# shangzhouye/stereo-visual-slam

Hardware: AMD Instinct MI355X
Metric: stereo keyframes/sec (ORB+match+tri+local-BA), KITTI-00 1241x376 (higher is better)
Workload: dtype u8+f64

## Files before the change

### stereo-visual-slam_amd/csrc/api.hip

```cpp
#include <stdarg.h>
#include <stdlib.h>

#include <algorithm>
#include <cmath>
#include <cfloat>
#include <cmath>
#include <vector>

#include "se3_device.h"
#include "vslam_internal.h"

#include <mutex>

namespace vslam {

static thread_local char g_err[512] = "";
void set_error(const char* fmt, ...) {
    va_list ap;
    va_start(ap, fmt);
    vsnprintf(g_err, sizeof(g_err), fmt, ap);
    va_end(ap);
}

struct Prof {
// ... 48 lines not shown
    c->stage_bytes = want; c->dev_bytes += want;
    return VSLAM_OK;
}
template <typename T>
static T* arena_take(Arena& a, size_t n) {
    a.off = (a.off + 255) & ~(size_t)255;
    T* p = reinterpret_cast<T*>(a.c->d_stage + a.off);
    a.off += n * sizeof(T);
    return p;
}
static size_t al256(size_t x) { return (x + 255) & ~(size_t)255; }

static CamParams cam_of(const Ctx* c) {
    CamParams cam;
    cam.fx = c->p.cam[0]; cam.fy = c->p.cam[1]; cam.cx = c->p.cam[2]; cam.cy = c->p.cam[3]; cam.b = c->p.cam[4];
    cam.dmin = c->p.depth_min; cam.dmax = c->p.depth_max; cam.drel = c->p.depth_reliable; cam.row_tol = c->p.stereo_row_tol;
    return cam;
}

template <typename T>
static int dev_alloc(Ctx* c, T** p, size_t n) {
    VS_HIP(hipMalloc((void**)p, n * sizeof(T)));
    c->dev_bytes += n * sizeof(T);
    return VSLAM_OK;
}

struct TuneKey { const char* name; const char* env; int Tuning::*field; int lo, hi; };
static const TuneKey kTuneKeys[] = {
    {"orb_fuse_min", "VSLAM_ORB_FUSE_MIN", &Tuning::orb_fuse_min, 0, 1 << 30},
    {"sgbm_fuse_min", "VSLAM_SGBM_FUSE_MIN", &Tuning::sgbm_fuse_min, 0, 1 << 30},
    {"sgbm_fwd_min", "VSLAM_SGBM_FWD_MIN", &Tuning::sgbm_fwd_min, 0, 1 << 30},
    {"sgbm_fw_rows", "VSLAM_SGBM_FW_ROWS", &Tuning::sgbm_fw_rows, 32, 64},
    {"pose_only_window", "VSLAM_POSE_ONLY_WINDOW", &Tuning::pose_only_window, 0, 1},
    {"ba_resident", "VSLAM_BA_RESIDENT", &Tuning::ba_resident, 0, 1},
    {"pnp_window", "VSLAM_PNP_WINDOW", &Tuning::pnp_window, 0, 1},
    {"ba_adaptive", "VSLAM_BA_ADAPTIVE", &Tuning::ba_adaptive, 0, 1},
    {"ba_lanes", "VSLAM_BA_LANES", &Tuning::ba_lanes, 256, 512},
    {"track_rule", "VSLAM_TRACK_RULE", &Tuning::track_rule, 0, 1},
};
static int tune_set(Tuning& t, const TuneKey& k, long v) {
    if (v == -1) { t.*(k.field) = -1; return VSLAM_OK; }
    if (v < k.lo || v > k.hi || (k.field == &Tuning::sgbm_fw_rows && v != 32 && v != 64) || (k.field == &Tuning::ba_lanes && v != 256 && v != 512)) {
        set_error("tuning value %s = %ld out of range (%d..%d%s, or -1 = default)", k.name, v, k.lo, k.hi, k.field == &Tuning::sgbm_fw_rows ? ", 32 or 64" : "");
        return VSLAM_ERR_ARG;
    }
    t.*(k.field) = (int)v;
    return VSLAM_OK;
}
static int tune_from_env(Tuning& t) {
    for (const TuneKey& k : kTuneKeys) {
        const char* e = getenv(k.env);
        if (!e || !*e) continue;
        char* end = nullptr;
        const long v = strtol(e, &end, 10);
        if (end == e || *end != 0) { set_error("environment variable %s = \"%s\" is not an integer", k.env, e); return VSLAM_ERR_ARG; }
        int rc = tune_set(t, k, v);
        if (rc) return rc;
    }
    return VSLAM_OK;
}

static int orb_status_check(Ctx* c, int B) {
    std::vector<int32_t> st(B);
    VS_HIP(hipMemcpyAsync(st.data(), c->orb.d_status, sizeof(int32_t) * B, hipMemcpyDeviceToHost, c->stream));
    VS_HIP(hipStreamSynchronize(c->stream));
    for (int b = 0; b < B; ++b)
// ... 1042 lines not shown
```

### stereo-visual-slam_amd/csrc/lm_kernels.hip

```cpp
#include "vslam_internal.h"

#include <stdlib.h>

#include <vector>

#include "se3_device.h"
#include "lm_device.h"

namespace vslam {

constexpr int kLmBlock = 512;
constexpr int kLmItemFixed = 128;
constexpr int kLmMinWaves = 2;
constexpr int kLmWaves = kLmBlock / 64;
constexpr int kMaxKf = VSLAM_MAX_KF;
constexpr int kMaxNp = 6 * kMaxKf;
constexpr int kMaxPairs = kMaxKf * (kMaxKf + 1) / 2;
constexpr int kHitsPerEdge = (kMaxKf + 1) / 2 + 1;
constexpr int kDinvLds = 1950;
constexpr int kLin = 2;
constexpr int kPoseParts = 3;
constexpr int kCntStride = 80;
constexpr int kItemSlots = (kMaxPairs + kLmWaves - 1) / kLmWaves;
constexpr int kDbgSlots = 24;
constexpr int kLmSlots = 5;
constexpr int kSchedFinalIters = 10;
constexpr int kRowCap = 512;

size_t lm_hits_per_edge() { return kHitsPerEdge; }

struct alignas(16) LmShared {
    double S[kMaxNp * kMaxNp];
    double Hpp[kMaxKf * 36], HppT[kMaxKf * 36];
    double bp[kMaxNp], bpT[kMaxNp], bs[kMaxNp], xp[kMaxNp];
    double rdiag[kMaxNp];
    double Ld[kMaxKf * 24];
// ... 4 lines not shown
    int ptot[kCntStride];
    int cnt[kLmWaves * kCntStride];
    uint8_t item[kLmWaves * kItemSlots];
    uint8_t pk1[kCntStride], pk2[kCntStride];
    int kfp[kMaxKf + 4];
    int rowp[kMaxKf + 4];
    int flag[8];
    int pairp[kMaxPairs + 2];
    uint8_t rowmax[kRowCap];
};
static_assert(kMaxKf * kPoseParts >= kMaxKf + kLmWaves - 1, "part[] must hold one slot per (keyframe, wave) segment");
static_assert(kLmWaves <= 16, "cnt rows");
static_assert(kMaxNp <= 128, "the backward substitution keeps two unknowns per lane of a wave");
static_assert(kMaxPairs <= kLmWaves * kItemSlots, "item[] too small");

struct LmKernelArgs {
    LmWindowArgs a;
    const int32_t* pnp_n;
    int capacity;
    uint8_t* act;
    int32_t* kf_pos;
    double* chi2k;
    float* uvk;
    int32_t* status;
    long long* dbg_cycles;
    float* slot_uv;
    uint8_t* slot_kf;
    uint8_t* lcnt;
    int dinv_lds;
    int want_chi2;
    const int32_t* order;
    int32_t* passes;
    const int32_t* defer;
};

__device__ inline int slot_width(const uint8_t* rowmax, int first) {
    const int row = first >> 6;
    return __builtin_amdgcn_readfirstlane(row < kRowCap ? (int)rowmax[min(row, kRowCap - 1)] : kLmSlots);
}

__device__ inline double block_sum(double v, double* red) {
    v = wave_sum(v);
    __syncthreads();
    if ((threadIdx.x & 63) == 0) red[threadIdx.x >> 6] = v;
    __syncthreads();
    double s = 0;
    for (int w = 0; w < kLmWaves; ++w) s += red[w];
    return s;
}
__device__ inline double block_max(double v, double* red) {
    v = wave_max(v);
    __syncthreads();
    if ((threadIdx.x & 63) == 0) red[threadIdx.x >> 6] = v;
    __syncthreads();
    double s = red[0];
    for (int w = 1; w < kLmWaves; ++w) s = fmax(s, red[w]);
    return s;
}

template <bool IMPL, bool SCHED = false>
__global__ __launch_bounds__(kLmBlock, kLmMinWaves) void lm_window_kernel(LmKernelArgs ka, int mode, int iters, int update_poses, int update_lms,
                                                            int classify, int reuse_csr) {
    static_assert(!(IMPL && SCHED), "the schedule is a property of the window problems");
    const LmWindowArgs& a = ka.a;
    __shared__ LmShared sm;
    const int w = ka.order ? ka.order[blockIdx.x] : (int)blockIdx.x;
// ... 1158 lines not shown
                currentChi = tempChi;
#pragma unroll
                for (int i = 0; i < 7; ++i) T[i] = Tt[i];
#pragma unroll
                for (int i = 0; i < 12; ++i) Rt[i] = Rtt[i];
            } else {
                lambda *= ni;
                ni *= 2;
            }
            ++qmax;
            again = (rho_gain < 0) && qmax < 10;
        }
        total_trials += qmax;
        if (st && lane == 0 && it < VSLAM_LM_MAX_ITERS) { st->chi2_iter[it] = currentChi; st->lambda_iter[it] = lambda; st->trials_iter[it] = qmax; }
        if (qmax == 10 || rho_gain == 0) { ++it; break; }
    }
    if (st && lane == 0) { st->iterations = it; st->total_trials = total_trials; st->chi2_final = currentChi; st->lambda_final = lambda; }
    if (lane < 7) d_T[7 * (size_t)b + lane] = T[lane];
    int mine = 0;
    for (int i = lane; i < n; i += 64) {
        const size_t gi = (size_t)b * capacity + i;
        double X, Y, Z, ex, ey;
        project_err(Rt, K, (double)px[3 * i], (double)px[3 * i + 1], (double)px[3 * i + 2], uv[2 * gi], uv[2 * gi + 1], X, Y, Z, ex, ey);
        const double c = ex * ex + ey * ey;
        const bool ok = isfinite(c) && c <= thr2;
        if (inlier) inlier[gi] = ok;
        mine += ok;
    }
    for (int o = 32; o > 0; o >>= 1) mine += __shfl_xor(mine, o);
    if (lane == 0 && n_inl) n_inl[b] = mine;
}

constexpr int kPoBlock = 64 * kMaxKf;
struct PoShared {
    double H[2][kMaxKf][36], g[2][kMaxKf][6];
    double part[2][kMaxKf], spart[2][kMaxKf];
    int cnt[kMaxKf][kMaxKf];
    int kbeg[kMaxKf + 1];
    int flag[2];
    int cin[2][kMaxKf], cout[2][kMaxKf];
    double T[2][kMaxKf][7], R[3][kMaxKf][12];
};
__global__ __launch_bounds__(kPoBlock) void pose_only_wave_kernel(LmKernelArgs ka, int iters, int update_poses) {
    const LmWindowArgs& a = ka.a;
    __shared__ PoShared sm;
    const int w = ka.order ? ka.order[blockIdx.x] : (int)blockIdx.x, tid = threadIdx.x, lane = tid & 63;
    const int wave = __builtin_amdgcn_readfirstlane(tid >> 6);
    if (ka.status[w] != VSLAM_OK) return;
    long long* cyc = ka.dbg_cycles ? ka.dbg_cycles + kDbgSlots * (size_t)w : nullptr;
    long long t_ph = cyc ? clock64() : 0;
#define POH(i) do { if (cyc && tid == 0) { const long long t1__ = clock64(); cyc[i] += t1__ - t_ph; t_ph = t1__; } } while (0)
    const int nk = a.n_kf_w ? min(max(a.n_kf_w[w], 1), a.n_kf) : a.n_kf;
    const int lm0 = a.lm_off[w], e0 = a.edge_off[w], ne = a.edge_off[w + 1] - e0;
    const int32_t* kfi = a.kf_idx + e0;
    const int32_t* lmi = a.lm_idx + e0;
    const float2* uv2 = reinterpret_cast<const float2*>(a.uv) + e0;
    const float* xyz = a.xyz + 3 * (size_t)lm0;
    uint8_t* inl = a.lm_inlier + lm0;
    int32_t* list = a.kf_edges + e0;
    float2* uvk = reinterpret_cast<float2*>(ka.uvk) + e0;
    float4* posk = reinterpret_cast<float4*>(a.lin) + e0;
    double* chik = ka.chi2k + e0;
    const double K[4] = {a.K[0], a.K[1], a.K[2], a.K[3]};
    const CamK ck = make_camk(K);
    const double delta = a.huber_delta;
    const unsigned long long lt_mask = (1ull << lane) - 1ull;
    const int per = (((ne + kMaxKf - 1) / kMaxKf) + 63) & ~63;
    const int c0 = min(wave * per, ne), c1 = min(c0 + per, ne);
    {
        int cnt[kMaxKf];
#pragma unroll
        for (int k = 0; k < kMaxKf; ++k) cnt[k] = 0;
        for (int base = c0; base < c1; base += 256) {
            int kq[4], lq[4]; bool vq[4]; uint8_t iq[4];
#pragma unroll
            for (int u = 0; u < 4; ++u) { const int e = base + 64 * u + lane; vq[u] = e < c1; const int es = min(e, ne - 1); kq[u] = kfi[es]; lq[u] = lmi[es]; }
#pragma unroll
            for (int u = 0; u < 4; ++u) iq[u] = inl[lq[u]];
#pragma unroll
            for (int u = 0; u < 4; ++u) {
                const bool act = vq[u] && iq[u] != 0;
#pragma unroll
                for (int kk = 0; kk < kMaxKf; ++kk) cnt[kk] += __popcll(__ballot(act && kq[u] == kk));
            }
        }
        if (lane < kMaxKf) {
            int v = 0;
#pragma unroll
            for (int kk = 0; kk < kMaxKf; ++kk) if (lane == kk) v = cnt[kk];
            sm.cnt[wave][lane] = v;
        }
        if (tid < 2) sm.flag[tid] = 0;
    }
    __syncthreads();
    int off[kMaxKf];
    {
        int run = 0;
#pragma unroll
        for (int k = 0; k < kMaxKf; ++k) {
            int before = 0, tot = 0;
#pragma unroll
            for (int c = 0; c < kMaxKf; ++c) { const int v = sm.cnt[c][k]; tot += v; if (c < wave) before += v; }
            off[k] = run + before;
            if (tid == 0) sm.kbeg[k] = run;
            run += tot;
        }
        if (tid == 0) sm.kbeg[kMaxKf] = run;
    }
    for (int base = c0; base < c1; base += 256) {
        int kq[4], lq[4], eq[4]; bool vq[4]; uint8_t iq[4]; float2 zq[4]; float Xq[4], Yq[4], Zq[4];
#pragma unroll
        for (int u = 0; u < 4; ++u) {
            const int e = base + 64 * u + lane; vq[u] = e < c1; eq[u] = e;
            const int es = min(e, ne - 1);
            kq[u] = kfi[es]; lq[u] = lmi[es]; zq[u] = uv2[es];
        }
#pragma unroll
        for (int u = 0; u < 4; ++u) { iq[u] = inl[lq[u]]; Xq[u] = xyz[3 * lq[u]]; Yq[u] = xyz[3 * lq[u] + 1]; Zq[u] = xyz[3 * lq[u] + 2]; }
#pragma unroll
        for (int u = 0; u < 4; ++u) {
            const bool act = vq[u] && iq[u] != 0;
#pragma unroll
            for (int kk = 0; kk < kMaxKf; ++kk) {
                const unsigned long long m = __ballot(act && kq[u] == kk);
                if (act && kq[u] == kk) {
                    const int pos = off[kk] + __popcll(m & lt_mask);
                    list[pos] = eq[u]; uvk[pos] = zq[u]; posk[pos] = make_float4(Xq[u], Yq[u], Zq[u], 0.f);
                }
                off[kk] += __popcll(m);
            }
        }
    }
    __syncthreads();
    POH(0);
    const int ntot = sm.kbeg[kMaxKf];
    const bool mine = wave < nk;
    const int kb = mine ? sm.kbeg[wave] : 0, ke = mine ? sm.kbeg[wave + 1] : 0;
    {
        double T[7], Rt[12];
#pragma unroll
        for (int i = 0; i < 7; ++i) T[i] = a.T[((size_t)w * a.n_kf + min(wave, nk - 1)) * 7 + i];
        expand_pose(T, Rt);
        if (lane == 0) {
#pragma unroll
            for (int i = 0; i < 7; ++i) sm.T[0][wave][i] = T[i];
#pragma unroll
            for (int i = 0; i < 12; ++i) { sm.R[0][wave][i] = Rt[i]; sm.R[2][wave][i] = Rt[i]; }
        }
        __builtin_amdgcn_wave_barrier();
    }
    const int slot27 = wave_slot<27>(lane);
    auto evaluate = [&](const double* Rlds, bool lin, int buf, bool store_chi) -> double {
        double R[12];
#pragma unroll
        for (int i = 0; i < 12; ++i) R[i] = uniform_f64(Rlds[i]);
        double part = 0, acc[27];
#pragma unroll
        for (int i = 0; i < 27; ++i) acc[i] = 0;
        float4 pp[2], pn[2]; float2 zz[2], zn[2];
#pragma unroll
        for (int u = 0; u < 2; ++u) { const int j = min(kb + 64 * u + lane, max(ke - 1, 0)); pp[u] = posk[j]; zz[u] = uvk[j]; }
        for (int j0 = kb; j0 < ke; j0 += 128) {
#pragma unroll
            for (int u = 0; u < 2; ++u) { const int j = min(j0 + 128 + 64 * u + lane, ke - 1); pn[u] = posk[j]; zn[u] = uvk[j]; }
#pragma unroll
            for (int u = 0; u < 2; ++u) {
                const int j = j0 + 64 * u + lane;
                if (j >= ke) continue;
                double x, y, ri, wgt, ex, ey, c, rho;
                cam_norm(R, (double)pp[u].x, (double)pp[u].y, (double)pp[u].z, x, y, ri);
                eval_obs(ck, x, y, zz[u], delta, ex, ey, c, rho, wgt);
                part += rho;
                if (store_chi) chik[j] = c;
                if (lin) {
                    double A[12], wA[12];
                    jac_norm(x, y, ri, A);
                    const double l0 = wgt * ck.fx2, l1 = wgt * ck.fy2;
#pragma unroll
                    for (int i = 0; i < 6; ++i) { wA[i] = l0 * A[i]; wA[6 + i] = l1 * A[6 + i]; }
                    int idx = 0;
#pragma unroll
                    for (int r = 0; r < 6; ++r)
#pragma unroll
                        for (int cc = r; cc < 6; ++cc) { acc[idx] = a_fma_pair(wA, r, A, cc, acc[idx]); ++idx; }
#pragma unroll
                    for (int r = 0; r < 6; ++r) acc[21 + r] = a_fma2(wA, r, -ex, -ey, acc[21 + r]);
                }
            }
#pragma unroll
            for (int u = 0; u < 2; ++u) { pp[u] = pn[u]; zz[u] = zn[u]; }
        }
        const double total = wave_sum(part);
        if (lin && mine) {
            wave_reduce_scatter<27>(acc, lane);
            if (slot27 >= 0 && slot27 < 21) {
                int r = 0, rem = slot27;
                while (rem >= 6 - r) { rem -= 6 - r; ++r; }
                const int cc = r + rem;
                sm.H[buf][wave][6 * r + cc] = acc[0]; sm.H[buf][wave][6 * cc + r] = acc[0];
            } else if (slot27 >= 21) sm.g[buf][wave][slot27 - 21] = acc[0];
        }
        return total;
    };
    auto sum_kf = [&](const double* v) -> double {
        double t = 0;
        for (int k = 0; k < nk; ++k) t += v[k];
        return t;
    };
    vslam_lm_stats* st = a.stats ? a.stats + w : nullptr;
    double lambda = 0, ni = 2, currentChi = 0;
    int pc = 0;
    int cur = 0, it = 0, total_trials = 0, pb = 0, fb = 0;
    if (iters > 0) {
        const double c = evaluate(sm.R[pc][wave], true, cur, false);
        if (lane == 0 && mine) sm.part[pb][wave] = c;
        __syncthreads();
        currentChi = sum_kf(sm.part[pb]);
        pb ^= 1;
        double md = 0;
        for (int k = 0; k < nk; ++k)
#pragma unroll
            for (int d = 0; d < 6; ++d) md = fmax(md, fabs(sm.H[cur][k][7 * d]));
        lambda = 1e-5 * md;
        if (st && tid == 0) st->chi2_init = currentChi;
    }
    POH(1);
    for (it = 0; it < iters; ++it) {
        double rho_gain = 0;
        int qmax = 0;
        bool again = true;
        while (again) {
            double x[6] = {0, 0, 0, 0, 0, 0};
            if (mine) {
                double Hk[36], gk[6];
#pragma unroll
                for (int i = 0; i < 36; ++i) Hk[i] = sm.H[cur][wave][i];
#pragma unroll
                for (int i = 0; i < 6; ++i) gk[i] = sm.g[cur][wave][i];
                if (!chol6_solve(Hk, lambda, gk, x) && lane == 0) sm.flag[fb] = 1;
            }
            POH(2);
            __syncthreads();
            POH(3);
            const bool ok2 = sm.flag[fb] == 0;
            if (tid == 0) sm.flag[fb ^ 1] = 0;
            fb ^= 1;
            if (!ok2) {
#pragma unroll
                for (int i = 0; i < 6; ++i) x[i] = 0;
            }
            {
                double E[7], Tc[7], Tt[7], Rtt[12];
#pragma unroll
                for (int i = 0; i < 7; ++i) Tc[i] = sm.T[pc][wave][i];
                se3::exp(x, E);
                se3::mul(E, Tc, Tt);
                expand_pose(Tt, Rtt);
                __builtin_amdgcn_wave_barrier();
                if (lane == 0) {
#pragma unroll
                    for (int i = 0; i < 7; ++i) sm.T[pc ^ 1][wave][i] = Tt[i];
#pragma unroll
                    for (int i = 0; i < 12; ++i) { sm.R[pc ^ 1][wave][i] = Rtt[i]; sm.R[2][wave][i] = Rtt[i]; }
                }
                __builtin_amdgcn_wave_barrier();
            }
            POH(4);
            const double c = evaluate(sm.R[pc ^ 1][wave], true, cur ^ 1, false);
            POH(5);
            double sc = 0;
            if (mine) {
#pragma unroll
                for (int i = 0; i < 6; ++i) sc += x[i] * (lambda * x[i] + sm.g[cur][wave][i]);
            }
            if (lane == 0 && mine) { sm.part[pb][wave] = c; sm.spart[pb][wave] = sc; }
            __syncthreads();
            POH(6);
            double tempChi = sum_kf(sm.part[pb]);
            const double scale = sum_kf(sm.spart[pb]) + 1e-3;
            pb ^= 1;
            if (!ok2) tempChi = 1.7976931348623157e308;
            rho_gain = (currentChi - tempChi) / scale;
            if (rho_gain > 0 && isfinite(tempChi)) {
                double alpha = 1. - pow(2 * rho_gain - 1, 3);
                alpha = fmin(alpha, 2. / 3.);
                lambda *= fmax(1. / 3., alpha);
                ni = 2;
                currentChi = tempChi;
                pc ^= 1;
                cur ^= 1;
            } else {
                lambda *= ni;
                ni *= 2;
            }
            ++qmax;
            again = (rho_gain < 0) && qmax < 10;
        }
        total_trials += qmax;
        if (st && tid == 0 && it < VSLAM_LM_MAX_ITERS) { st->chi2_iter[it] = currentChi; st->lambda_iter[it] = lambda; st->trials_iter[it] = qmax; }
        if (qmax == 10 || rho_gain == 0) { ++it; break; }
    }
    if (st && tid == 0) { st->iterations = it; st->total_trials = total_trials; st->chi2_final = currentChi; st->lambda_final = lambda; }
    POH(7);
    evaluate(sm.R[2][wave], false, 0, true);
    double th = delta;
    int cb = 0;
    for (int iteration = 0; iteration < 5; ++iteration) {
        int cin = 0, cout = 0;
        for (int j = kb + lane; j < ke; j += 64) { if (chik[j] > th) ++cout; else ++cin; }
        for (int o = 32; o > 0; o >>= 1) { cin += __shfl_xor(cin, o); cout += __shfl_xor(cout, o); }
        if (lane == 0) { sm.cin[cb][wave] = mine ? cin : 0; sm.cout[cb][wave] = mine ? cout : 0; }
        __syncthreads();
        int tin = 0, tout = 0;
        for (int k = 0; k < nk; ++k) { tin += sm.cin[cb][k]; tout += sm.cout[cb][k]; }
        cb ^= 1;
        const double ratio = (double)tin / (double)(tin + tout);
        if (ratio > 0.5) break;
        th *= 2;
    }
    if (ka.want_chi2) {
        double* chi2 = a.chi2 + e0;
        for (int e = tid; e < ne; e += kPoBlock) if (!inl[lmi[e]]) chi2[e] = 0.0;
        for (int j = kb + lane; j < ke; j += 64) chi2[list[j]] = chik[j];
    }
    __syncthreads();
    for (int j = kb + lane; j < ke; j += 64) {
        const int e = list[j];
        if (e == ne - 1 || lmi[e + 1] != lmi[e]) inl[lmi[e]] = !(chik[j] > th);
    }
    if (tid == 0 && a.chi2_thr) a.chi2_thr[w] = th;
    if (update_poses && mine && lane < 7) a.T[((size_t)w * a.n_kf + wave) * 7 + lane] = sm.T[pc][wave][lane];
    POH(8);
    (void)ntot;
#undef POH
}

static int ensure(void** p, size_t* have, size_t need) {
    if (*have >= need) return VSLAM_OK;
    if (*p) hipFree(*p);
    *p = nullptr; *have = 0;
    if (hipMalloc(p, need) != hipSuccess) { set_error("LM scratch hipMalloc(%zu) failed", need); return VSLAM_ERR_HIP; }
    *have = need;
    return VSLAM_OK;
}

static int carve(LmScratch& g_lm, LmKernelArgs& ka, size_t total_lm, size_t total_edge, int n_windows, bool with_lm, hipStream_t stream) {
    auto al = [](size_t x) { return (x + 255) & ~(size_t)255; };
    size_t need = 0;
    const size_t o_P = need; need += al(total_lm * 3 * 8);
    const size_t o_Pt = need; need += al(total_lm * 3 * 8);
    const size_t o_Hll = need; need += al(total_lm * 6 * 8);
    const size_t o_bl = need; need += al(total_lm * 3 * 8);
    const size_t o_Di = need; need += al(total_lm * 6 * 8);
    const size_t o_lin = need; need += al(total_edge * kLin * 8);
    const size_t o_lmptr = need; need += al((total_lm + n_windows + 1) * 4);
    const size_t o_kfptr = need; need += al((size_t)n_windows * (kMaxKf + 1) * 4);
    const size_t o_kfe = need; need += al(total_edge * 4);
    const size_t o_pp = need; need += al((size_t)n_windows * (kMaxPairs + 1) * 4);
    const size_t o_hits = need; need += with_lm ? al(total_edge * kHitsPerEdge * 8) : 256;
    const size_t o_act = need; need += al(total_lm);
    const size_t o_kpos = need; need += al(total_edge * 4);
    const size_t o_st = need; need += al((size_t)n_windows * 4);
    const size_t o_chi = need; need += al(total_edge * 8);
    const size_t o_chik = need; need += al(total_edge * 8);
    const size_t o_uvk = need; need += al(total_edge * 8);
    const size_t o_suv = need; need += with_lm ? al(total_lm * kLmSlots * 8) : 256;
// ... 83 lines not shown
        L.dyn_bytes = scratch->rs_dyn_bytes; L.schedule = schedule; L.adaptive = adaptive ? 1 : 0; L.iters = iters; L.update_poses = update_poses; L.update_lms = update_lms;
        L.opt_in_done = scratch->rs_opt_in; L.want_chi2 = ka.want_chi2;
        L.dense_to_general = !(scratch->tune && scratch->tune->ba_resident == 1);
        if (schedule && !adaptive) hipLaunchKernelGGL(lm_fill_kernel, dim3((a.n_windows + 255) / 256), dim3(256), 0, stream, ka.passes, a.n_windows, 3);
        rc = launch_ba_resident(L, stream);
        if (rc) return rc;
        scratch->rs_opt_in = true;
        ka.defer = scratch->defer;
        if (L.dbg) {
            hipStreamSynchronize(stream);
            std::vector<long long> h(kDbgSlots * (size_t)a.n_windows);
            hipMemcpy(h.data(), ka.dbg_cycles, sizeof(long long) * h.size(), hipMemcpyDeviceToHost);
            static const char* rs_names[16] = {"setup", "pass init", "boot evaluation", "lambda-init pass", "linearise", "convert+cholesky+solve", "pose update+backsub+trial eval",
                                               "(loop tail)", "classification", "write-back", "lin: row open", "lin: landmark blocks", "lin: diag pair (row-wise)", "lin: off-diag pairs (row-wise)", "lin: singles chunks", "(classification: row loop)"};
            double tot = 0;
            for (int i = 0; i < 16; ++i) { double sum = 0; for (int w = 0; w < a.n_windows; ++w) sum += (double)h[16 * (size_t)w + i]; sum /= a.n_windows; if (i < 10) tot += sum; fprintf(stderr, "  [rs profile] %-32s %10.0f ticks/window\n", rs_names[i], sum); }
            fprintf(stderr, "  [rs profile] total %.0f (clock64 ticks)\n", tot);
            hipMemsetAsync(ka.dbg_cycles, 0, sizeof(long long) * kDbgSlots * a.n_windows, stream);
        }
    }
    if (schedule) {
        if (adaptive) {
            hipLaunchKernelGGL((lm_window_kernel<false, true>), dim3(a.n_windows), dim3(kLmBlock), dyn_lds, stream, ka, 0, 5, 0, 0, 1, 0);
        } else {
            if (!resident) hipLaunchKernelGGL(lm_fill_kernel, dim3((a.n_windows + 255) / 256), dim3(256), 0, stream, ka.passes, a.n_windows, 3);
            hipLaunchKernelGGL(lm_window_kernel<false>, dim3(a.n_windows), dim3(kLmBlock), dyn_lds, stream, ka, 0, 5, 0, 0, 1, 0);
            hipLaunchKernelGGL(lm_window_kernel<false>, dim3(a.n_windows), dim3(kLmBlock), dyn_lds, stream, ka, 0, 5, 0, 0, 1, 1);
            hipLaunchKernelGGL(lm_window_kernel<false>, dim3(a.n_windows), dim3(kLmBlock), dyn_lds, stream, ka, 0, kSchedFinalIters, 1, 0, 1, 1);
        }
        ka.defer = nullptr;
        const bool po_window = scratch->tune && scratch->tune->pose_only_window > 0;
        if (po_window) hipLaunchKernelGGL(lm_window_kernel<false>, dim3(a.n_windows), dim3(kLmBlock), dyn_lds, stream, ka, 1, 10, 1, 0, 1, resident ? 0 : 1);
        else {
            if (ka.dbg_cycles && getenv("VSLAM_PO_PROFILE")) hipMemsetAsync(ka.dbg_cycles, 0, sizeof(long long) * kDbgSlots * a.n_windows, stream);
            hipLaunchKernelGGL(pose_only_wave_kernel, dim3(a.n_windows), dim3(kPoBlock), 0, stream, ka, 10, 1);
        }
    } else {
        hipLaunchKernelGGL(lm_window_kernel<false>, dim3(a.n_windows), dim3(kLmBlock), dyn_lds, stream, ka, mode, iters, update_poses, update_lms, 1, 0);
    }
    VS_HIP(hipGetLastError());
    if (ka.dbg_cycles) {
        hipStreamSynchronize(stream);
        std::vector<long long> h(kDbgSlots * (size_t)a.n_windows);
        hipMemcpy(h.data(), ka.dbg_cycles, sizeof(long long) * h.size(), hipMemcpyDeviceToHost);
        static const char* names[kDbgSlots] = {"setup", "eval+lin", "lm blocks", "pose blocks", "lambda/Dinv", "bs", "schur", "cholesky (rest)", "solve (rest)", "update+scale", "eval trial", "loop tail", "classify+wb", "(setup: csr)", "(setup: kf-major)", "schur: item prologue",
                                               "chol: diag+rows", "chol: barrier 1", "chol: trailing update", "chol: barrier 2", "solve: barrier", "solve: back-subst", "schur: rows", "schur: reduce+store"};
        double tot = 0;
        for (int i = 0; i < kDbgSlots; ++i) { double s = 0; for (int w = 0; w < a.n_windows; ++w) s += (double)h[kDbgSlots * (size_t)w + i]; s /= a.n_windows; if (i < 13 || i >= 16) tot += s; fprintf(stderr, "  [lm profile] %-20s %10.0f ticks/window\n", names[i], s); }
        fprintf(stderr, "  [lm profile] total %.0f cycles (clock64 = shader clock, thread 0 of every window; setup sub-splits not included)\n", tot);
    }
    return VSLAM_OK;
}

int lm_fetch_deferred(const LmScratch* scratch, int n_windows, int32_t* h_defer, hipStream_t stream) {
    if (!scratch->buf || !scratch->defer || !h_defer || n_windows > scratch->status_n) return VSLAM_ERR_ARG;
    if (!scratch->defer_valid) { for (int w = 0; w < n_windows; ++w) h_defer[w] = 1; return VSLAM_OK; }
    VS_HIP(hipMemcpyAsync(h_defer, scratch->defer, sizeof(int32_t) * n_windows, hipMemcpyDeviceToHost, stream));
    VS_HIP(hipStreamSynchronize(stream));
    for (int w = 0; w < n_windows; ++w) h_defer[w] &= 1;
    return VSLAM_OK;
}

int lm_fetch_passes(const LmScratch* scratch, int n_windows, int32_t* h_passes, hipStream_t stream) {
    if (!scratch->buf || !scratch->passes || !h_passes || n_windows > scratch->status_n) return VSLAM_ERR_ARG;
    VS_HIP(hipMemcpyAsync(h_passes, scratch->passes, sizeof(int32_t) * n_windows, hipMemcpyDeviceToHost, stream));
    VS_HIP(hipStreamSynchronize(stream));
    return VSLAM_OK;
}

int lm_fetch_status(const LmScratch* scratch, int n_windows, int32_t* h_status, hipStream_t stream) {
    const LmScratch& g_lm = *scratch;
    if (!g_lm.buf || !h_status) return VSLAM_ERR_ARG;
    VS_HIP(hipMemcpyAsync(h_status, g_lm.status, sizeof(int32_t) * n_windows, hipMemcpyDeviceToHost, stream));
    VS_HIP(hipStreamSynchronize(stream));
    return VSLAM_OK;
}

// ... 65 lines not shown
```

### stereo-visual-slam_amd/csrc/vslam_internal.h

```cpp
#pragma once
#include <hip/hip_runtime.h>
#include <stdint.h>
#include <stdio.h>
#include <string.h>

#include "../../include/vslam_hip.h"

namespace vslam {

void set_error(const char* fmt, ...);

#define VS_HIP(call)                                                                              \
    do {                                                                                          \
        hipError_t e__ = (call);                                                                  \
        if (e__ != hipSuccess) {                                                                  \
            ::vslam::set_error("%s:%d %s -> %s", __FILE__, __LINE__, #call, hipGetErrorString(e__)); \
            return VSLAM_ERR_HIP;                                                                 \
        }                                                                                         \
    } while (0)

struct Prof;
Prof* prof_current();
void prof_set_current(Prof* p);
void prof_begin(hipStream_t s, const char* name, int launches);
// ... 119 lines not shown
    const int32_t* edge_off;
    double* T;
    float* xyz;
    const uint8_t* reliable;
    uint8_t* lm_inlier;
    const int32_t* kf_idx;
    const int32_t* lm_idx;
    const float* uv;
    double* chi2;
    vslam_lm_stats* stats;
    double* P;
    double* Ptrial;
    double* Hll;
    double* bl;
    double* Dinv;
    double* lin;
    int32_t* lm_ptr;
    int32_t* kf_ptr;
    int32_t* kf_edges;
    int32_t* pair_ptr;
    int32_t* pair_hits;
    int32_t hit_capacity_per_edge;
    double K[4];
    double huber_delta;
    double* chi2_thr;
    size_t total_lm, total_edge;
};
struct Tuning {
    int orb_fuse_min = -1;
    int sgbm_fuse_min = -1;
    int sgbm_fwd_min = -1;
    int sgbm_fw_rows = -1;
    int pose_only_window = -1;
    int pnp_window = -1;
    int ba_lanes = -1;
    int ba_resident = -1;
    int track_rule = -1;
    int ba_adaptive = -1;
};
int launch_sgbm(const Tuning& tune, const uint8_t* d_left, const uint8_t* d_right, size_t img_bytes, int pitch, int w, int h, int B, float* d_disp_f32,
                int16_t* d_disp_i16, int16_t* d_disp_raw, uint8_t** scratch, size_t* scratch_bytes, size_t* dev_bytes, hipStream_t stream);
size_t sgbm_scratch_bytes(int w, int h, int B);

struct LmScratch {
    void* buf = nullptr; size_t bytes = 0;
    int32_t* status = nullptr; int status_n = 0;
    int32_t* passes = nullptr;
    const Tuning* tune = nullptr;
    bool lds_opt_in = false;
    bool rs_opt_in = false;
    int rs_dyn_bytes = -1;
    int32_t* defer = nullptr;
    bool defer_valid = false;
};
struct RsLaunch {
    LmWindowArgs a;
    void* uv_s; int32_t* epos; double* tab; double* xin; double* Pbak; double* Dc; double* blc;
    int32_t* status; int32_t* passes; int32_t* defer; const int32_t* order; long long* dbg;
    int dyn_bytes, schedule, adaptive, iters, update_poses, update_lms, dense_to_general;
    int want_chi2;
    int lanes;
    bool opt_in_done;
};
int rs_dyn_lds_bytes(int device);
int launch_ba_resident(const RsLaunch& L, hipStream_t stream);
int launch_lm_windows(const LmWindowArgs& a, int schedule, int mode, int iters, int update_poses, int update_lms, LmScratch* scratch,
                      hipStream_t stream);
size_t lm_hits_per_edge();
int lm_fetch_status(const LmScratch* scratch, int n_windows, int32_t* h_status, hipStream_t stream);
int lm_fetch_passes(const LmScratch* scratch, int n_windows, int32_t* h_passes, hipStream_t stream);
int lm_fetch_deferred(const LmScratch* scratch, int n_windows, int32_t* h_defer, hipStream_t stream);

struct PnpArgs {
    const float* xyz; const float* uv; const int32_t* n; int capacity; int B;
    double* T; int iters; double K[4]; double huber_delta; double reproj_thr;
    uint8_t* inlier; int32_t* n_inliers; vslam_lm_stats* stats;
    int n_hint;
};
int launch_pnp(const PnpArgs& a, LmScratch* scratch, hipStream_t stream);
int launch_edge_jacobians(int n, const float* d_xyz, const float* d_uv, const double* d_T, const double K[4], double delta, double* d_err, double* d_Jp, double* d_Jl,
                          double* d_chi2, double* d_hw, hipStream_t stream);
size_t pnp_epnp_ws_bytes(int H);
int launch_pnp_epnp(const float* d_hx, const float* d_hu, int H, const double K[4], double* d_Rt, double* d_T, int32_t* d_ok, uint8_t* ws, hipStream_t stream);
// ... 34 lines not shown
```

Baseline: 61480.

## Stage pose-only LM edge runs in dynamic LDS instead of global scratch

The pose-only wave kernel now bucketizes per-keyframe edge data (observations, 3D points, edge ids, chi2) into dynamically sized shared memory when the window's active edge count fits. The evaluate loop, which runs many times per LM iteration, then reads from LDS rather than global scratch. It falls back to the global-memory path for oversized windows. Requesting the maximum dynamic LDS per block may reduce occupancy, and the code adds a tuning knob and profiling output.

```diff
diff --git a/stereo-visual-slam_amd/csrc/api.hip b/stereo-visual-slam_amd/csrc/api.hip
--- a/stereo-visual-slam_amd/csrc/api.hip
+++ b/stereo-visual-slam_amd/csrc/api.hip
@@ -104,6 +104,7 @@
     {"sgbm_fwd_min", "VSLAM_SGBM_FWD_MIN", &Tuning::sgbm_fwd_min, 0, 1 << 30},
     {"sgbm_fw_rows", "VSLAM_SGBM_FW_ROWS", &Tuning::sgbm_fw_rows, 32, 64},
     {"pose_only_window", "VSLAM_POSE_ONLY_WINDOW", &Tuning::pose_only_window, 0, 1},
+    {"pose_only_lds_edges", "VSLAM_POSE_ONLY_LDS_EDGES", &Tuning::pose_only_lds_edges, 0, 1 << 30},
     {"ba_resident", "VSLAM_BA_RESIDENT", &Tuning::ba_resident, 0, 1},
     {"pnp_window", "VSLAM_PNP_WINDOW", &Tuning::pnp_window, 0, 1},
     {"ba_adaptive", "VSLAM_BA_ADAPTIVE", &Tuning::ba_adaptive, 0, 1},
diff --git a/stereo-visual-slam_amd/csrc/lm_kernels.hip b/stereo-visual-slam_amd/csrc/lm_kernels.hip
--- a/stereo-visual-slam_amd/csrc/lm_kernels.hip
+++ b/stereo-visual-slam_amd/csrc/lm_kernels.hip
@@ -2,6 +2,7 @@
 
 #include <stdlib.h>
 
+#include <type_traits>
 #include <vector>
 
 #include "se3_device.h"
@@ -72,6 +73,7 @@
     const int32_t* order;
     int32_t* passes;
     const int32_t* defer;
+    int po_cap;
 };
 
 __device__ inline int slot_width(const uint8_t* rowmax, int first) {
@@ -1296,6 +1298,30 @@
 }
 
 constexpr int kPoBlock = 64 * kMaxKf;
+constexpr int kPoEdgeBytes = 24;
+struct PoRunsGlobal {
+    static constexpr bool kAhead = true;
+    int32_t* list; float2* uvk; float4* posk; double* chik;
+    __device__ void put(int p, int e, float2 z, float X, float Y, float Z) const { list[p] = e; uvk[p] = z; posk[p] = make_float4(X, Y, Z, 0.f); }
+    __device__ float4 pos(int j) const { return posk[j]; }
+    __device__ float2 obs(int j) const { return uvk[j]; }
+    __device__ void set_chi(int j, double c) const { chik[j] = c; }
+    __device__ double chi(int j) const { return chik[j]; }
+    __device__ int edge(int j) const { return list[j]; }
+};
+struct PoRunsLds {
+    static constexpr bool kAhead = false;
+    unsigned long long* oz; float *x, *y, *z; int32_t* id;
+    __device__ void put(int p, int e, float2 o, float X, float Y, float Z) const {
+        oz[p] = (unsigned long long)__float_as_uint(o.x) | ((unsigned long long)__float_as_uint(o.y) << 32);
+        x[p] = X; y[p] = Y; z[p] = Z; id[p] = e;
+    }
+    __device__ float4 pos(int j) const { return make_float4(x[j], y[j], z[j], 0.f); }
+    __device__ float2 obs(int j) const { const unsigned long long v = oz[j]; return make_float2(__uint_as_float((unsigned)v), __uint_as_float((unsigned)(v >> 32))); }
+    __device__ void set_chi(int j, double c) const { oz[j] = (unsigned long long)__double_as_longlong(c); }
+    __device__ double chi(int j) const { return __longlong_as_double((long long)oz[j]); }
+    __device__ int edge(int j) const { return id[j]; }
+};
 struct PoShared {
     double H[2][kMaxKf][36], g[2][kMaxKf][6];
     double part[2][kMaxKf], spart[2][kMaxKf];
@@ -1308,6 +1334,7 @@
 __global__ __launch_bounds__(kPoBlock) void pose_only_wave_kernel(LmKernelArgs ka, int iters, int update_poses) {
     const LmWindowArgs& a = ka.a;
     __shared__ PoShared sm;
+    extern __shared__ unsigned long long po_dyn[];
     const int w = ka.order ? ka.order[blockIdx.x] : (int)blockIdx.x, tid = threadIdx.x, lane = tid & 63;
     const int wave = __builtin_amdgcn_readfirstlane(tid >> 6);
     if (ka.status[w] != VSLAM_OK) return;
@@ -1321,10 +1348,6 @@
     const float2* uv2 = reinterpret_cast<const float2*>(a.uv) + e0;
     const float* xyz = a.xyz + 3 * (size_t)lm0;
     uint8_t* inl = a.lm_inlier + lm0;
-    int32_t* list = a.kf_edges + e0;
-    float2* uvk = reinterpret_cast<float2*>(ka.uvk) + e0;
-    float4* posk = reinterpret_cast<float4*>(a.lin) + e0;
-    double* chik = ka.chi2k + e0;
     const double K[4] = {a.K[0], a.K[1], a.K[2], a.K[3]};
     const CamK ck = make_camk(K);
     const double delta = a.huber_delta;
@@ -1358,6 +1381,7 @@
     }
     __syncthreads();
     int off[kMaxKf];
+    int ntot;
     {
         int run = 0;
 #pragma unroll
@@ -1370,232 +1394,249 @@
             run += tot;
         }
         if (tid == 0) sm.kbeg[kMaxKf] = run;
-    }
-    for (int base = c0; base < c1; base += 256) {
-        int kq[4], lq[4], eq[4]; bool vq[4]; uint8_t iq[4]; float2 zq[4]; float Xq[4], Yq[4], Zq[4];
-#pragma unroll
-        for (int u = 0; u < 4; ++u) {
-            const int e = base + 64 * u + lane; vq[u] = e < c1; eq[u] = e;
-            const int es = min(e, ne - 1);
-            kq[u] = kfi[es]; lq[u] = lmi[es]; zq[u] = uv2[es];
-        }
-#pragma unroll
-        for (int u = 0; u < 4; ++u) { iq[u] = inl[lq[u]]; Xq[u] = xyz[3 * lq[u]]; Yq[u] = xyz[3 * lq[u] + 1]; Zq[u] = xyz[3 * lq[u] + 2]; }
-#pragma unroll
-        for (int u = 0; u < 4; ++u) {
-            const bool act = vq[u] && iq[u] != 0;
-#pragma unroll
-            for (int kk = 0; kk < kMaxKf; ++kk) {
-                const unsigned long long m = __ballot(act && kq[u] == kk);
-                if (act && kq[u] == kk) {
-                    const int pos = off[kk] + __popcll(m & lt_mask);
-                    list[pos] = eq[u]; uvk[pos] = zq[u]; posk[pos] = make_float4(Xq[u], Yq[u], Zq[u], 0.f);
-                }
-                off[kk] += __popcll(m);
-            }
-        }
-    }
-    __syncthreads();
-    POH(0);
-    const int ntot = sm.kbeg[kMaxKf];
-    const bool mine = wave < nk;
-    const int kb = mine ? sm.kbeg[wave] : 0, ke = mine ? sm.kbeg[wave + 1] : 0;
-    {
-        double T[7], Rt[12];
-#pragma unroll
-        for (int i = 0; i < 7; ++i) T[i] = a.T[((size_t)w * a.n_kf + min(wave, nk - 1)) * 7 + i];
-        expand_pose(T, Rt);
-        if (lane == 0) {
-#pragma unroll
-            for (int i = 0; i < 7; ++i) sm.T[0][wave][i] = T[i];
-#pragma unroll
-            for (int i = 0; i < 12; ++i) { sm.R[0][wave][i] = Rt[i]; sm.R[2][wave][i] = Rt[i]; }
-        }
-        __builtin_amdgcn_wave_barrier();
-    }
-    const int slot27 = wave_slot<27>(lane);
-    auto evaluate = [&](const double* Rlds, bool lin, int buf, bool store_chi) -> double {
-        double R[12];
-#pragma unroll
-        for (int i = 0; i < 12; ++i) R[i] = uniform_f64(Rlds[i]);
-        double part = 0, acc[27];
-#pragma unroll
-        for (int i = 0; i < 27; ++i) acc[i] = 0;
-        float4 pp[2], pn[2]; float2 zz[2], zn[2];
-#pragma unroll
-        for (int u = 0; u < 2; ++u) { const int j = min(kb + 64 * u + lane, max(ke - 1, 0)); pp[u] = posk[j]; zz[u] = uvk[j]; }
-        for (int j0 = kb; j0 < ke; j0 += 128) {
-#pragma unroll
-            for (int u = 0; u < 2; ++u) { const int j = min(j0 + 128 + 64 * u + lane, ke - 1); pn[u] = posk[j]; zn[u] = uvk[j]; }
-#pragma unroll
-            for (int u = 0; u < 2; ++u) {
-                const int j = j0 + 64 * u + lane;
-                if (j >= ke) continue;
-                double x, y, ri, wgt, ex, ey, c, rho;
-                cam_norm(R, (double)pp[u].x, (double)pp[u].y, (double)pp[u].z, x, y, ri);
-                eval_obs(ck, x, y, zz[u], delta, ex, ey, c, rho, wgt);
-                part += rho;
-                if (store_chi) chik[j] = c;
-                if (lin) {
-                    double A[12], wA[12];
-                    jac_norm(x, y, ri, A);
-                    const double l0 = wgt * ck.fx2, l1 = wgt * ck.fy2;
-#pragma unroll
-                    for (int i = 0; i < 6; ++i) { wA[i] = l0 * A[i]; wA[6 + i] = l1 * A[6 + i]; }
-                    int idx = 0;
-#pragma unroll
-                    for (int r = 0; r < 6; ++r)
-#pragma unroll
-                        for (int cc = r; cc < 6; ++cc) { acc[idx] = a_fma_pair(wA, r, A, cc, acc[idx]); ++idx; }
-#pragma unroll
-                    for (int r = 0; r < 6; ++r) acc[21 + r] = a_fma2(wA, r, -ex, -ey, acc[21 + r]);
-                }
-            }
-#pragma unroll
-            for (int u = 0; u < 2; ++u) { pp[u] = pn[u]; zz[u] = zn[u]; }
-        }
-        const double total = wave_sum(part);
-        if (lin && mine) {
-            wave_reduce_scatter<27>(acc, lane);
-            if (slot27 >= 0 && slot27 < 21) {
-                int r = 0, rem = slot27;
-                while (rem >= 6 - r) { rem -= 6 - r; ++r; }
-                const int cc = r + rem;
-                sm.H[buf][wave][6 * r + cc] = acc[0]; sm.H[buf][wave][6 * cc + r] = acc[0];
-            } else if (slot27 >= 21) sm.g[buf][wave][slot27 - 21] = acc[0];
-        }
-        return total;
+        ntot = __builtin_amdgcn_readfirstlane(run);
+    }
+    auto body = [&](const auto& S) {
+        for (int base = c0; base < c1; base += 256) {
+            int kq[4], lq[4], eq[4]; bool vq[4]; uint8_t iq[4]; float2 zq[4]; float Xq[4], Yq[4], Zq[4];
+#pragma unroll
+            for (int u = 0; u < 4; ++u) {
+                const int e = base + 64 * u + lane; vq[u] = e < c1; eq[u] = e;
+                const int es = min(e, ne - 1);
+                kq[u] = kfi[es]; lq[u] = lmi[es]; zq[u] = uv2[es];
+            }
+#pragma unroll
+            for (int u = 0; u < 4; ++u) { iq[u] = inl[lq[u]]; Xq[u] = xyz[3 * lq[u]]; Yq[u] = xyz[3 * lq[u] + 1]; Zq[u] = xyz[3 * lq[u] + 2]; }
+#pragma unroll
+            for (int u = 0; u < 4; ++u) {
+                const bool act = vq[u] && iq[u] != 0;
+#pragma unroll
+                for (int kk = 0; kk < kMaxKf; ++kk) {
+                    const unsigned long long m = __ballot(act && kq[u] == kk);
+                    if (act && kq[u] == kk) {
+                        const int pos = off[kk] + __popcll(m & lt_mask);
+                        S.put(pos, eq[u], zq[u], Xq[u], Yq[u], Zq[u]);
+                    }
+                    off[kk] += __popcll(m);
+                }
+            }
+        }
+        __syncthreads();
+        POH(0);
+        const bool mine = wave < nk;
+        const int kb = mine ? sm.kbeg[wave] : 0, ke = mine ? sm.kbeg[wave + 1] : 0;
+        {
+            double T[7], Rt[12];
+#pragma unroll
+            for (int i = 0; i < 7; ++i) T[i] = a.T[((size_t)w * a.n_kf + min(wave, nk - 1)) * 7 + i];
+            expand_pose(T, Rt);
+            if (lane == 0) {
+#pragma unroll
+                for (int i = 0; i < 7; ++i) sm.T[0][wave][i] = T[i];
+#pragma unroll
+                for (int i = 0; i < 12; ++i) { sm.R[0][wave][i] = Rt[i]; sm.R[2][wave][i] = Rt[i]; }
+            }
+            __builtin_amdgcn_wave_barrier();
+        }
+        const int slot27 = wave_slot<27>(lane);
+        auto evaluate = [&](const double* Rlds, bool lin, int buf, bool store_chi) -> double {
+            double R[12];
+#pragma unroll
+            for (int i = 0; i < 12; ++i) R[i] = uniform_f64(Rlds[i]);
+            double part = 0, acc[27];
+#pragma unroll
+            for (int i = 0; i < 27; ++i) acc[i] = 0;
+            constexpr bool ahead = std::decay_t<decltype(S)>::kAhead;
+            float4 pp[2], pn[2]; float2 zz[2], zn[2];
+            if constexpr (ahead) {
+#pragma unroll
+                for (int u = 0; u < 2; ++u) { const int j = min(kb + 64 * u + lane, max(ke - 1, 0)); pp[u] = S.pos(j); zz[u] = S.obs(j); }
+            }
+            for (int j0 = kb; j0 < ke; j0 += 128) {
+#pragma unroll
+                for (int u = 0; u < 2; ++u) {
+                    if constexpr (ahead) { const int j = min(j0 + 128 + 64 * u + lane, ke - 1); pn[u] = S.pos(j); zn[u] = S.obs(j); }
+                    else { const int j = min(j0 + 64 * u + lane, ke - 1); pp[u] = S.pos(j); zz[u] = S.obs(j); }
+                }
+#pragma unroll
+                for (int u = 0; u < 2; ++u) {
+                    const int j = j0 + 64 * u + lane;
+                    if (j >= ke) continue;
+                    double x, y, ri, wgt, ex, ey, c, rho;
+                    cam_norm(R, (double)pp[u].x, (double)pp[u].y, (double)pp[u].z, x, y, ri);
+                    eval_obs(ck, x, y, zz[u], delta, ex, ey, c, rho, wgt);
+                    part += rho;
+                    if (store_chi) S.set_chi(j, c);
+                    if (lin) {
+                        double A[12], wA[12];
+                        jac_norm(x, y, ri, A);
+                        const double l0 = wgt * ck.fx2, l1 = wgt * ck.fy2;
+#pragma unroll
+                        for (int i = 0; i < 6; ++i) { wA[i] = l0 * A[i]; wA[6 + i] = l1 * A[6 + i]; }
+                        int idx = 0;
+#pragma unroll
+                        for (int r = 0; r < 6; ++r)
+#pragma unroll
+                            for (int cc = r; cc < 6; ++cc) { acc[idx] = a_fma_pair(wA, r, A, cc, acc[idx]); ++idx; }
+#pragma unroll
+                        for (int r = 0; r < 6; ++r) acc[21 + r] = a_fma2(wA, r, -ex, -ey, acc[21 + r]);
+                    }
+                }
+                if constexpr (ahead) {
+#pragma unroll
+                    for (int u = 0; u < 2; ++u) { pp[u] = pn[u]; zz[u] = zn[u]; }
+                }
+            }
+            const double total = wave_sum(part);
+            if (lin && mine) {
+                wave_reduce_scatter<27>(acc, lane);
+                if (slot27 >= 0 && slot27 < 21) {
+                    int r = 0, rem = slot27;
+                    while (rem >= 6 - r) { rem -= 6 - r; ++r; }
+                    const int cc = r + rem;
+                    sm.H[buf][wave][6 * r + cc] = acc[0]; sm.H[buf][wave][6 * cc + r] = acc[0];
+                } else if (slot27 >= 21) sm.g[buf][wave][slot27 - 21] = acc[0];
+            }
+            return total;
+        };
+        auto sum_kf = [&](const double* v) -> double {
+            double t = 0;
+            for (int k = 0; k < nk; ++k) t += v[k];
+            return t;
+        };
+        vslam_lm_stats* st = a.stats ? a.stats + w : nullptr;
+        double lambda = 0, ni = 2, currentChi = 0;
+        int pc = 0;
+        int cur = 0, it = 0, total_trials = 0, pb = 0, fb = 0;
+        if (iters > 0) {
+            const double c = evaluate(sm.R[pc][wave], true, cur, false);
+            if (lane == 0 && mine) sm.part[pb][wave] = c;
+            __syncthreads();
+            currentChi = sum_kf(sm.part[pb]);
+            pb ^= 1;
+            double md = 0;
+            for (int k = 0; k < nk; ++k)
+#pragma unroll
+                for (int d = 0; d < 6; ++d) md = fmax(md, fabs(sm.H[cur][k][7 * d]));
+            lambda = 1e-5 * md;
+            if (st && tid == 0) st->chi2_init = currentChi;
+        }
+        POH(1);
+        for (it = 0; it < iters; ++it) {
+            double rho_gain = 0;
+            int qmax = 0;
+            bool again = true;
+            while (again) {
+                double x[6] = {0, 0, 0, 0, 0, 0};
+                if (mine) {
+                    double Hk[36], gk[6];
+#pragma unroll
+                    for (int i = 0; i < 36; ++i) Hk[i] = sm.H[cur][wave][i];
+#pragma unroll
+                    for (int i = 0; i < 6; ++i) gk[i] = sm.g[cur][wave][i];
+                    if (!chol6_solve(Hk, lambda, gk, x) && lane == 0) sm.flag[fb] = 1;
+                }
+                POH(2);
+                __syncthreads();
+                POH(3);
+                const bool ok2 = sm.flag[fb] == 0;
+                if (tid == 0) sm.flag[fb ^ 1] = 0;
+                fb ^= 1;
+                if (!ok2) {
+#pragma unroll
+                    for (int i = 0; i < 6; ++i) x[i] = 0;
+                }
+                {
+                    double E[7], Tc[7], Tt[7], Rtt[12];
+#pragma unroll
+                    for (int i = 0; i < 7; ++i) Tc[i] = sm.T[pc][wave][i];
+                    se3::exp(x, E);
+                    se3::mul(E, Tc, Tt);
+                    expand_pose(Tt, Rtt);
+                    __builtin_amdgcn_wave_barrier();
+                    if (lane == 0) {
+#pragma unroll
+                        for (int i = 0; i < 7; ++i) sm.T[pc ^ 1][wave][i] = Tt[i];
+#pragma unroll
+                        for (int i = 0; i < 12; ++i) { sm.R[pc ^ 1][wave][i] = Rtt[i]; sm.R[2][wave][i] = Rtt[i]; }
+                    }
+                    __builtin_amdgcn_wave_barrier();
+                }
+                POH(4);
+                const double c = evaluate(sm.R[pc ^ 1][wave], true, cur ^ 1, false);
+                POH(5);
+                double sc = 0;
+                if (mine) {
+#pragma unroll
+                    for (int i = 0; i < 6; ++i) sc += x[i] * (lambda * x[i] + sm.g[cur][wave][i]);
+                }
+                if (lane == 0 && mine) { sm.part[pb][wave] = c; sm.spart[pb][wave] = sc; }
+                __syncthreads();
+                POH(6);
+                double tempChi = sum_kf(sm.part[pb]);
+                const double scale = sum_kf(sm.spart[pb]) + 1e-3;
+                pb ^= 1;
+                if (!ok2) tempChi = 1.7976931348623157e308;
+                rho_gain = (currentChi - tempChi) / scale;
+                if (rho_gain > 0 && isfinite(tempChi)) {
+                    double alpha = 1. - pow(2 * rho_gain - 1, 3);
+                    alpha = fmin(alpha, 2. / 3.);
+                    lambda *= fmax(1. / 3., alpha);
+                    ni = 2;
+                    currentChi = tempChi;
+                    pc ^= 1;
+                    cur ^= 1;
+                } else {
+                    lambda *= ni;
+                    ni *= 2;
+                }
+                ++qmax;
+                again = (rho_gain < 0) && qmax < 10;
+            }
+            total_trials += qmax;
+            if (st && tid == 0 && it < VSLAM_LM_MAX_ITERS) { st->chi2_iter[it] = currentChi; st->lambda_iter[it] = lambda; st->trials_iter[it] = qmax; }
+            if (qmax == 10 || rho_gain == 0) { ++it; break; }
+        }
+        if (st && tid == 0) { st->iterations = it; st->total_trials = total_trials; st->chi2_final = currentChi; st->lambda_final = lambda; }
+        POH(7);
+        evaluate(sm.R[2][wave], false, 0, true);
+        double th = delta;
+        int cb = 0;
+        for (int iteration = 0; iteration < 5; ++iteration) {
+            int cin = 0, cout = 0;
+            for (int j = kb + lane; j < ke; j += 64) { if (S.chi(j) > th) ++cout; else ++cin; }
+            for (int o = 32; o > 0; o >>= 1) { cin += __shfl_xor(cin, o); cout += __shfl_xor(cout, o); }
+            if (lane == 0) { sm.cin[cb][wave] = mine ? cin : 0; sm.cout[cb][wave] = mine ? cout : 0; }
+            __syncthreads();
+            int tin = 0, tout = 0;
+            for (int k = 0; k < nk; ++k) { tin += sm.cin[cb][k]; tout += sm.cout[cb][k]; }
+            cb ^= 1;
+            const double ratio = (double)tin / (double)(tin + tout);
+            if (ratio > 0.5) break;
+            th *= 2;
+        }
+        if (ka.want_chi2) {
+            double* chi2 = a.chi2 + e0;
+            for (int e = tid; e < ne; e += kPoBlock) if (!inl[lmi[e]]) chi2[e] = 0.0;
+            for (int j = kb + lane; j < ke; j += 64) chi2[S.edge(j)] = S.chi(j);
+        }
+        __syncthreads();
+        for (int j = kb + lane; j < ke; j += 64) {
+            const int e = S.edge(j);
+            if (e == ne - 1 || lmi[e + 1] != lmi[e]) inl[lmi[e]] = !(S.chi(j) > th);
+        }
+        if (tid == 0 && a.chi2_thr) a.chi2_thr[w] = th;
+        if (update_poses && mine && lane < 7) a.T[((size_t)w * a.n_kf + wave) * 7 + lane] = sm.T[pc][wave][lane];
+        POH(8);
     };
-    auto sum_kf = [&](const double* v) -> double {
-        double t = 0;
-        for (int k = 0; k < nk; ++k) t += v[k];
-        return t;
-    };
-    vslam_lm_stats* st = a.stats ? a.stats + w : nullptr;
-    double lambda = 0, ni = 2, currentChi = 0;
-    int pc = 0;
-    int cur = 0, it = 0, total_trials = 0, pb = 0, fb = 0;
-    if (iters > 0) {
-        const double c = evaluate(sm.R[pc][wave], true, cur, false);
-        if (lane == 0 && mine) sm.part[pb][wave] = c;
-        __syncthreads();
-        currentChi = sum_kf(sm.part[pb]);
-        pb ^= 1;
-        double md = 0;
-        for (int k = 0; k < nk; ++k)
-#pragma unroll
-            for (int d = 0; d < 6; ++d) md = fmax(md, fabs(sm.H[cur][k][7 * d]));
-        lambda = 1e-5 * md;
-        if (st && tid == 0) st->chi2_init = currentChi;
-    }
-    POH(1);
-    for (it = 0; it < iters; ++it) {
-        double rho_gain = 0;
-        int qmax = 0;
-        bool again = true;
-        while (again) {
-            double x[6] = {0, 0, 0, 0, 0, 0};
-            if (mine) {
-                double Hk[36], gk[6];
-#pragma unroll
-                for (int i = 0; i < 36; ++i) Hk[i] = sm.H[cur][wave][i];
-#pragma unroll
-                for (int i = 0; i < 6; ++i) gk[i] = sm.g[cur][wave][i];
-                if (!chol6_solve(Hk, lambda, gk, x) && lane == 0) sm.flag[fb] = 1;
-            }
-            POH(2);
-            __syncthreads();
-            POH(3);
-            const bool ok2 = sm.flag[fb] == 0;
-            if (tid == 0) sm.flag[fb ^ 1] = 0;
-            fb ^= 1;
-            if (!ok2) {
-#pragma unroll
-                for (int i = 0; i < 6; ++i) x[i] = 0;
-            }
-            {
-                double E[7], Tc[7], Tt[7], Rtt[12];
-#pragma unroll
-                for (int i = 0; i < 7; ++i) Tc[i] = sm.T[pc][wave][i];
-                se3::exp(x, E);
-                se3::mul(E, Tc, Tt);
-                expand_pose(Tt, Rtt);
-                __builtin_amdgcn_wave_barrier();
-                if (lane == 0) {
-#pragma unroll
-                    for (int i = 0; i < 7; ++i) sm.T[pc ^ 1][wave][i] = Tt[i];
-#pragma unroll
-                    for (int i = 0; i < 12; ++i) { sm.R[pc ^ 1][wave][i] = Rtt[i]; sm.R[2][wave][i] = Rtt[i]; }
-                }
-                __builtin_amdgcn_wave_barrier();
-            }
-            POH(4);
-            const double c = evaluate(sm.R[pc ^ 1][wave], true, cur ^ 1, false);
-            POH(5);
-            double sc = 0;
-            if (mine) {
-#pragma unroll
-                for (int i = 0; i < 6; ++i) sc += x[i] * (lambda * x[i] + sm.g[cur][wave][i]);
-            }
-            if (lane == 0 && mine) { sm.part[pb][wave] = c; sm.spart[pb][wave] = sc; }
-            __syncthreads();
-            POH(6);
-            double tempChi = sum_kf(sm.part[pb]);
-            const double scale = sum_kf(sm.spart[pb]) + 1e-3;
-            pb ^= 1;
-            if (!ok2) tempChi = 1.7976931348623157e308;
-            rho_gain = (currentChi - tempChi) / scale;
-            if (rho_gain > 0 && isfinite(tempChi)) {
-                double alpha = 1. - pow(2 * rho_gain - 1, 3);
-                alpha = fmin(alpha, 2. / 3.);
-                lambda *= fmax(1. / 3., alpha);
-                ni = 2;
-                currentChi = tempChi;
-                pc ^= 1;
-                cur ^= 1;
-            } else {
-                lambda *= ni;
-                ni *= 2;
-            }
-            ++qmax;
-            again = (rho_gain < 0) && qmax < 10;
-        }
-        total_trials += qmax;
-        if (st && tid == 0 && it < VSLAM_LM_MAX_ITERS) { st->chi2_iter[it] = currentChi; st->lambda_iter[it] = lambda; st->trials_iter[it] = qmax; }
-        if (qmax == 10 || rho_gain == 0) { ++it; break; }
-    }
-    if (st && tid == 0) { st->iterations = it; st->total_trials = total_trials; st->chi2_final = currentChi; st->lambda_final = lambda; }
-    POH(7);
-    evaluate(sm.R[2][wave], false, 0, true);
-    double th = delta;
-    int cb = 0;
-    for (int iteration = 0; iteration < 5; ++iteration) {
-        int cin = 0, cout = 0;
-        for (int j = kb + lane; j < ke; j += 64) { if (chik[j] > th) ++cout; else ++cin; }
-        for (int o = 32; o > 0; o >>= 1) { cin += __shfl_xor(cin, o); cout += __shfl_xor(cout, o); }
-        if (lane == 0) { sm.cin[cb][wave] = mine ? cin : 0; sm.cout[cb][wave] = mine ? cout : 0; }
-        __syncthreads();
-        int tin = 0, tout = 0;
-        for (int k = 0; k < nk; ++k) { tin += sm.cin[cb][k]; tout += sm.cout[cb][k]; }
-        cb ^= 1;
-        const double ratio = (double)tin / (double)(tin + tout);
-        if (ratio > 0.5) break;
-        th *= 2;
-    }
-    if (ka.want_chi2) {
-        double* chi2 = a.chi2 + e0;
-        for (int e = tid; e < ne; e += kPoBlock) if (!inl[lmi[e]]) chi2[e] = 0.0;
-        for (int j = kb + lane; j < ke; j += 64) chi2[list[j]] = chik[j];
-    }
-    __syncthreads();
-    for (int j = kb + lane; j < ke; j += 64) {
-        const int e = list[j];
-        if (e == ne - 1 || lmi[e + 1] != lmi[e]) inl[lmi[e]] = !(chik[j] > th);
-    }
-    if (tid == 0 && a.chi2_thr) a.chi2_thr[w] = th;
-    if (update_poses && mine && lane < 7) a.T[((size_t)w * a.n_kf + wave) * 7 + lane] = sm.T[pc][wave][lane];
-    POH(8);
-    (void)ntot;
+    const int cap = ka.po_cap;
+    if (ntot <= cap) {
+        float* x = reinterpret_cast<float*>(po_dyn + cap);
+        body(PoRunsLds{po_dyn, x, x + cap, x + 2 * cap, reinterpret_cast<int32_t*>(x + 3 * cap)});
+    } else {
+        if (cyc && tid == 0) cyc[9] += 1;
+        body(PoRunsGlobal{a.kf_edges + e0, reinterpret_cast<float2*>(ka.uvk) + e0, reinterpret_cast<float4*>(a.lin) + e0, ka.chi2k + e0});
+    }
 #undef POH
 }
 
@@ -1745,8 +1786,18 @@
         const bool po_window = scratch->tune && scratch->tune->pose_only_window > 0;
         if (po_window) hipLaunchKernelGGL(lm_window_kernel<false>, dim3(a.n_windows), dim3(kLmBlock), dyn_lds, stream, ka, 1, 10, 1, 0, 1, resident ? 0 : 1);
         else {
+            if (scratch->po_dyn_bytes < 0) {
+                int dev = 0, v = 0;
+                (void)hipGetDevice(&dev);
+                if (hipDeviceGetAttribute(&v, hipDeviceAttributeMaxSharedMemoryPerBlock, dev) != hipSuccess || v <= 0) v = 64 * 1024;
+                const int avail = v - (int)sizeof(PoShared) - 256;
+                scratch->po_dyn_bytes = avail > 0 ? avail & ~255 : 0;
+                VS_HIP(hipFuncSetAttribute(reinterpret_cast<const void*>(&pose_only_wave_kernel), hipFuncAttributeMaxDynamicSharedMemorySize, scratch->po_dyn_bytes));
+            }
+            ka.po_cap = scratch->po_dyn_bytes / kPoEdgeBytes;
+            if (scratch->tune && scratch->tune->pose_only_lds_edges >= 0) ka.po_cap = min(ka.po_cap, scratch->tune->pose_only_lds_edges);
             if (ka.dbg_cycles && getenv("VSLAM_PO_PROFILE")) hipMemsetAsync(ka.dbg_cycles, 0, sizeof(long long) * kDbgSlots * a.n_windows, stream);
-            hipLaunchKernelGGL(pose_only_wave_kernel, dim3(a.n_windows), dim3(kPoBlock), 0, stream, ka, 10, 1);
+            hipLaunchKernelGGL(pose_only_wave_kernel, dim3(a.n_windows), dim3(kPoBlock), (size_t)ka.po_cap * kPoEdgeBytes, stream, ka, 10, 1);
         }
     } else {
         hipLaunchKernelGGL(lm_window_kernel<false>, dim3(a.n_windows), dim3(kLmBlock), dyn_lds, stream, ka, mode, iters, update_poses, update_lms, 1, 0);
@@ -1756,6 +1807,11 @@
         hipStreamSynchronize(stream);
         std::vector<long long> h(kDbgSlots * (size_t)a.n_windows);
         hipMemcpy(h.data(), ka.dbg_cycles, sizeof(long long) * h.size(), hipMemcpyDeviceToHost);
+        if (schedule && getenv("VSLAM_PO_PROFILE") && !(scratch->tune && scratch->tune->pose_only_window > 0)) {
+            static const char* po_names[10] = {"setup", "initial evaluation", "6x6 solve", "barrier 1", "pose update", "trial evaluation", "barrier 2",
+                                               "loop tail", "classify+write-back", "(windows on the global path)"};
+            for (int i = 0; i < 10; ++i) { double s = 0; for (int w = 0; w < a.n_windows; ++w) s += (double)h[kDbgSlots * (size_t)w + i]; fprintf(stderr, "  [po profile] %-30s %12.2f %s\n", po_names[i], i < 9 ? s / a.n_windows : s, i < 9 ? "ticks/window" : "windows"); }
+        }
         static const char* names[kDbgSlots] = {"setup", "eval+lin", "lm blocks", "pose blocks", "lambda/Dinv", "bs", "schur", "cholesky (rest)", "solve (rest)", "update+scale", "eval trial", "loop tail", "classify+wb", "(setup: csr)", "(setup: kf-major)", "schur: item prologue",
                                                "chol: diag+rows", "chol: barrier 1", "chol: trailing update", "chol: barrier 2", "solve: barrier", "solve: back-subst", "schur: rows", "schur: reduce+store"};
         double tot = 0;
diff --git a/stereo-visual-slam_amd/csrc/vslam_internal.h b/stereo-visual-slam_amd/csrc/vslam_internal.h
--- a/stereo-visual-slam_amd/csrc/vslam_internal.h
+++ b/stereo-visual-slam_amd/csrc/vslam_internal.h
@@ -175,6 +175,7 @@
     int sgbm_fwd_min = -1;
     int sgbm_fw_rows = -1;
     int pose_only_window = -1;
+    int pose_only_lds_edges = -1;
     int pnp_window = -1;
     int ba_lanes = -1;
     int ba_resident = -1;
@@ -192,6 +193,7 @@
     const Tuning* tune = nullptr;
     bool lds_opt_in = false;
     bool rs_opt_in = false;
+    int po_dyn_bytes = -1;
     int rs_dyn_bytes = -1;
     int32_t* defer = nullptr;
     bool defer_valid = false;
```

Result: no change. 62160, median of 6 (+1.1%).
